# francescobrigante/Audio-Style-Transfer

Measured on AMD Instinct MI355X. Metric: audio-seconds/sec/node (train step, 4s@22.05kHz pairs), higher is better.
Workload: dtype bf16; 1 GPU; configs[1]: batch=8 4 s clips per GPU (S=2, x=(B,S,2,287,597)), full train2 step: STFT + CQT front-end from resident waveforms, encoders+decoder+discriminator, all losses, D and G phases, grad clip, Adam; global_batch=8, parallelism=dp1, hip_graph=True, dp_semantics=per-rank BN and batch-coupled losses

## Files before the change

### audio-style-transfer_amd/ast_amd/ops.py

```python
from __future__ import annotations

import functools
import math

import torch

from . import _lib, config
from ._lib import Gather, check, dcode, lib, ptr, stream


@functools.lru_cache(maxsize=None)
def const_tensor(values, dtype, device):
    return torch.tensor(values, dtype=dtype, device=device)


def pad8(c: int) -> int:
    return (c + 7) // 8 * 8


def _tap(dh, dw, wt):
    return (dh + 64) | ((dw + 64) << 8) | (wt << 16)


def _mk(N, Hs, Ws, Cs, Hm, Wm, sh, sw, oh, ow, Hd, Wd, Cd, dsh, dsw, doh, dow, taps, wtaps):
# ... 19 lines not shown
        th = [((ph + pad - kh) // stride, kh) for kh in range(k) if (ph + pad - kh) % stride == 0]
        Hm = (Hd - ph + stride - 1) // stride
        for pw in range(stride):
            tw = [((pw + pad - kw) // stride, kw) for kw in range(k) if (pw + pad - kw) % stride == 0]
            Wm = (Wd - pw + stride - 1) // stride
            if Hm <= 0 or Wm <= 0:
                continue
            taps = tuple((dh, dw, kh * k + kw) for dh, kh in th for dw, kw in tw)
            out.append(_mk(N, Hs, Ws, Cs, Hm, Wm, 1, 1, 0, 0, Hd, Wd, Cd, stride, stride, ph, pw, taps, k * k))
    return tuple(out)


PROFILE = None


def _gemm_cost(g, esize, wgrad=False):
    M = g.N * g.Hm * g.Wm
    K = g.ntaps * g.Cs
    flops = 2.0 * M * g.Cd * K
    if wgrad:
        nbytes = (M * g.Cd + g.N * g.Hs * g.Ws * g.Cs) * esize + g.Cd * K * 4
    else:
        src_pix = min(g.N * g.Hs * g.Ws, M * max(g.ntaps, 1))
        nbytes = (src_pix * g.Cs + M * g.Cd + g.Cd * K) * esize
    return flops, nbytes


def _igemm_config(g, dt):
    import ctypes
    out = (ctypes.c_int32 * 5)()
    check(lib().ast_igemm_plan(g, dt, ctypes.byref(out)), "ast_igemm_plan")
    if out[2] < 0:
        return f"patch{-out[0]}r{'(rows,' + str(-out[3]) + 'frag)' if out[3] < 0 else ''},{out[1]}ch,slab{-out[2]}B"
    return f"{out[0]}x{out[1]},k{out[2] * 16}B" + (f",split{out[3]}" if out[3] > 1 else "") + (f",kg{out[4]}" if out[4] > 1 else "")


_ws_cache = {}


def _ws_need(g, dt):
    key = (id(g), dt)
    v = _ws_cache.get(key)
    if v is None:
        v = int(lib().ast_igemm_ws_floats(g, dt))
        if v < 0:
            check(-1, "ast_igemm_ws_floats")
        _ws_cache[key] = v
    return v


STAT_SLOTS = 64


def stat_slots(C):
    s = STAT_SLOTS
    while s > 8 and s * C > 4096:
        s //= 2
    return s


def _slot_flags(slots):
    return 0 if slots == 64 else ((slots.bit_length() - 1) << 8)


class _StatArena:
    CAP = 1 << 24
# ... 13 lines not shown
        a[0].zero_()
        a[1] = 0
    t = a[0][a[1]:a[1] + int(n)]
    a[1] += n64
    a[2] = max(a[2], a[1])
    return t


def stat_arena_reset(device):
    a = _StatArena.by_device.get(torch.device(device))
    if a is None or a[2] == 0:
        return
    if config.fused_finalize or _SyncBN.active:
        a[0][:a[2]].zero_()
    a[1] = 0


def stats_fusable(g, dt):
    return _ws_need(g, dt) == 0


class BNLink:
    __slots__ = ("x", "scale", "shift", "relu", "table", "filled", "slots")

    def __init__(self):
        self.x = self.scale = self.shift = self.table = None
        self.relu, self.filled, self.slots = True, False, STAT_SLOTS


def in_stats_fusable(g, dt):
    import ctypes
    out = (ctypes.c_int32 * 5)()
    check(lib().ast_igemm_plan(g, dt, ctypes.byref(out)), "ast_igemm_plan")
    return out[2] != 0 and _ws_need(g, dt) == 0


def _igemm(src, wgt, bias, dst, g, flags=0, stats=None, bn=None, per_image=False):
    if PROFILE is not None:
        e0, e1 = torch.cuda.Event(enable_timing=True), torch.cuda.Event(enable_timing=True)
        e0.record()
    need = _ws_need(g, dcode(src.dtype))
    if bn is not None:
        assert need == 0 and flags == 0
        check(lib().ast_igemm_bn(ptr(src), ptr(wgt), ptr(bias), ptr(dst), g, dcode(src.dtype), 16 | (0 if bn.relu else 32) | _slot_flags(bn.slots), ptr(bn.table),
                                 bn.table.numel(), ptr(bn.x), ptr(bn.scale), ptr(bn.shift), stream()), "ast_igemm_bn")
    else:
        if stats is not None:
            assert need == 0 and flags == 0
            ws, need, flags = stats, stats.numel(), (8 | 64 if per_image else 8 | _slot_flags(stats.numel() // (2 * g.Cd)))
        else:
            ws = _clean_scratch(need, src.device) if need > 0 else None
            flags |= 4 if need > 0 else 0
        check(lib().ast_igemm(ptr(src), ptr(wgt), ptr(bias), ptr(dst), g, dcode(src.dtype), flags, ptr(ws), need,
                              stream()), "ast_igemm")
    if PROFILE is not None:
        e1.record()
        fl, by = _gemm_cost(g, src.element_size())
        dt = "bf16" if src.dtype == torch.bfloat16 else "f32"
        PROFILE.append((f"igemm_kernel<{dt},{_igemm_config(g, dcode(src.dtype))}>", fl, by, e0, e1))


class _WgradStream:
    stream = None
    dirty = False


def _wgrad(dy, src, dwp, g, replicas=1, pw=None):
# ... 1108 lines not shown
```

### audio-style-transfer_amd/csrc/igemm.hip

```cpp
#include "gemm_common.h"

namespace {


__device__ __forceinline__ int swz(int row, int c) { return ((c + (((row >> 3) & 1) << 1)) & 3) << 4; }

template <typename T>
struct EpiCtx {
  T* dst; const float* bias; float* ws; const T* bn_x; const float* bn_scale; const float* bn_shift;
  int HWm; float rcp_hw, rcp_w; bool accumulate, relu, stats, bstats, bn_relu;
};

template <typename T, int TN, int MODE>
__device__ __forceinline__ void epi_store_m(const EpiCtx<T>& ec, const ast_gather_t& g, const f32x4 (&col)[TN], const size_t pix, const int co0,
                                            float (&st1)[TN][4], float (&st2)[TN][4]) {
  T* drow = ec.dst + pix * g.Cd;
#pragma unroll
  for (int i = 0; i < TN; ++i) {
    const int co = co0 + i * 16;
    if (co >= g.Cd) continue;
    float v[4];
#pragma unroll
    for (int r = 0; r < 4; ++r) v[r] = col[i][r];
    if (ec.bias) {
// ... 310 lines not shown
  const bool split = gridDim.z > 1;
  const bool stats = (flags & 8) && !split;
  const bool bstats = (flags & 16) && !split;
  const bool bn_relu = !(flags & 32);
  EpiCtx<T> ec{dst, bias, ws, bn_x, bn_scale, bn_shift, HWm, rcp_hw, rcp_w, accumulate, relu, stats, bstats, bn_relu};
  float st1[TN][4], st2[TN][4];
#pragma unroll
  for (int i = 0; i < TN; ++i)
#pragma unroll
    for (int r = 0; r < 4; ++r) { st1[i][r] = 0.f; st2[i][r] = 0.f; }
#pragma unroll
  for (int j = 0; j < TM; ++j) {
    const int m = bm0 + wm * WTM + j * 16 + fr;
    if (m >= M_end) continue;
    if (split) {
#pragma unroll
      for (int i = 0; i < TN; ++i) {
        const int co = bn0 + wn * WTN + i * 16 + fq * 4;
        if (co >= g.Cd) continue;
#pragma unroll
        for (int r = 0; r < 4; ++r) unsafeAtomicAdd(ws + (size_t)m * g.Cd + co + r, acc[i][j][r]);
      }
      continue;
    }
    f32x4 col[TN];
#pragma unroll
    for (int i = 0; i < TN; ++i) col[i] = acc[i][j];
    epi_pixel<T, TN>(ec, g, col, m, bn0 + wn * WTN + fq * 4, st1, st2);
  }
  float* const red = (KG == 1 && WN == 1) ? reinterpret_cast<float*>(lds_all) : nullptr;
  if (stats || bstats) epi_flush<T, TN>(ec, g, st1, st2, per_image ? ~img : (tix & stat_slot_mask(flags)), bn0 + wn * WTN, fr, fq, red);
}

template <typename T, int TN, int NKS>
__global__ __launch_bounds__(256) void igemm_direct_kernel(const T* __restrict__ src, const T* __restrict__ wgt,
                                                           const float* __restrict__ bias, T* __restrict__ dst,
                                                           const ast_gather_t g, const int M, const int flags,
                                                           float* __restrict__ ws, const int cpc_shift,
                                                           const unsigned src_bytes, const unsigned wgt_bytes,
                                                           const float rcp_hw, const float rcp_w,
                                                           const T* __restrict__ bn_x, const float* __restrict__ bn_scale,
                                                           const float* __restrict__ bn_shift, const int jt) {
  constexpr int E = 16 / sizeof(T), ES = sizeof(T);
  constexpr unsigned OOB = 0x80000000u;
  using frag = typename Mma<T>::frag;
  __shared__ int taptab[AST_MAX_TAPS];
  const int lane = threadIdx.x & 63, wave = threadIdx.x >> 6;
  const int fr = lane & 15, fq = lane >> 4;
  const int BMW = jt * 16, BM = 4 * BMW;
  const int MT = (M + BM - 1) / BM, NT = (g.Cd + TN * 16 - 1) / (TN * 16);
  const int chunk = gridDim.x >> 3;
  const int tix = (blockIdx.x & 7) * chunk + (blockIdx.x >> 3);
  if (tix >= MT * NT) return;
  const int ntile = tix / MT;
  const int bm0 = (tix - ntile * MT) * BM + wave * BMW, bn0 = ntile * TN * 16;
#pragma unroll
  for (int t = 0; t < AST_MAX_TAPS; ++t)
    if ((int)threadIdx.x == t) taptab[t] = g.tap[t];
  __syncthreads();
  const int cpc = g.Cs / E, nchunks = g.ntaps * cpc;
  const int nks = (nchunks + 3) >> 2;
  const int HWm = g.Hm * g.Wm;
  const __amdgpu_buffer_rsrc_t srcR = __builtin_amdgcn_make_buffer_rsrc((void*)src, 0, src_bytes, 0x00020000);
  const __amdgpu_buffer_rsrc_t wgtR = __builtin_amdgcn_make_buffer_rsrc((void*)wgt, 0, wgt_bytes, 0x00020000);

  int sdelta[NKS], tdh[NKS], tdw[NKS];
  unsigned woff[NKS];
#pragma unroll
  for (int ks = 0; ks < NKS; ++ks) {
    const int kc = ks * 4 + fq;
    const bool kval = kc < nchunks;
    const int t = kval ? (cpc_shift >= 0 ? (kc >> cpc_shift) : kc / cpc) : 0;
    const int c0b = (kc - t * cpc) * 16;
    int dh, dw, wt;
    decode_tap(taptab[t], dh, dw, wt);
    sdelta[ks] = (dh * g.Ws + dw) * g.Cs * ES + c0b;
    tdh[ks] = kval ? dh : (1 << 20);
    tdw[ks] = dw;
    woff[ks] = kval ? (unsigned)(wt * g.Cs * ES + c0b) : OOB;
  }
  frag wreg[TN][NKS];
#pragma unroll
  for (int i = 0; i < TN; ++i) {
    const int co = bn0 + i * 16 + fr;
    const unsigned rowoff = co < g.Cd ? (unsigned)(co * g.wtaps * g.Cs * ES) : OOB;
#pragma unroll
    for (int ks = 0; ks < NKS; ++ks)
      wreg[i][ks] = __builtin_bit_cast(frag, __builtin_amdgcn_raw_buffer_load_b128(wgtR, (rowoff != OOB && woff[ks] != OOB) ? rowoff + woff[ks] : OOB, 0, 0));
  }

  const bool accumulate = flags & 1, relu = flags & 2, stats = flags & 8, bstats = flags & 16, bn_relu = !(flags & 32);
  EpiCtx<T> ec{dst, bias, ws, bn_x, bn_scale, bn_shift, HWm, rcp_hw, rcp_w, accumulate, relu, stats, bstats, bn_relu};
  float st1[TN][4], st2[TN][4];
#pragma unroll
  for (int i = 0; i < TN; ++i)
#pragma unroll
    for (int r = 0; r < 4; ++r) { st1[i][r] = 0.f; st2[i][r] = 0.f; }

  auto load_pix = [&](int j, u32x4 (&xr)[NKS], int& dpix) __attribute__((always_inline)) {
    const int m = bm0 + j * 16 + fr;
    const bool valid = j < jt && m < M;
    const int mm = valid ? m : 0;
    const int n = fdiv(mm, HWm, rcp_hw), rem = mm - n * HWm;
    const int hm = fdiv(rem, g.Wm, rcp_w), wq = rem - hm * g.Wm;
    const int hs0 = valid ? hm * g.sh + g.oh : -(1 << 20);
    const int ws0 = wq * g.sw + g.ow;
    const int roff = (((n * g.Hs + (valid ? hs0 : 0)) * g.Ws + ws0) * g.Cs) * ES;
    dpix = (n * g.Hd + hm * g.dsh + g.doh) * g.Wd + (wq * g.dsw + g.dow);
#pragma unroll
    for (int ks = 0; ks < NKS; ++ks) {
      const bool ok = (unsigned)(hs0 + tdh[ks]) < (unsigned)g.Hs && (unsigned)(ws0 + tdw[ks]) < (unsigned)g.Ws;
      xr[ks] = __builtin_amdgcn_raw_buffer_load_b128(srcR, ok ? (unsigned)(roff + sdelta[ks]) : OOB, 0, 0);
    }
  };
  auto compute = [&](int j, const u32x4 (&xr)[NKS], const int dpix) __attribute__((always_inline)) {
    f32x4 acc[TN];
#pragma unroll
    for (int i = 0; i < TN; ++i) acc[i] = f32x4{0.f, 0.f, 0.f, 0.f};
#pragma unroll
    for (int ks = 0; ks < NKS; ++ks) {
      if (ks < nks) {
        const frag xf = __builtin_bit_cast(frag, xr[ks]);
#pragma unroll
        for (int i = 0; i < TN; ++i) acc[i] = Mma<T>::run(wreg[i][ks], xf, acc[i]);
      }
    }
    const int m = bm0 + j * 16 + fr;
    if (m < M) epi_store<T, TN>(ec, g, acc, (size_t)dpix, bn0 + fq * 4, st1, st2);
  };

  u32x4 xa[NKS], xb[NKS];
  int pa, pb;
  load_pix(0, xa, pa);
  for (int j = 0; j < jt; j += 2) {
    load_pix(j + 1, xb, pb);
    compute(j, xa, pa);
    load_pix(j + 2, xa, pa);
    if (j + 1 < jt) compute(j + 1, xb, pb);
  }
  __shared__ float red[(TN + 1) / 2 * 256];
  if (stats || bstats) epi_flush<T, TN>(ec, g, st1, st2, tix & stat_slot_mask(flags), bn0, fr, fq, red);
}

template <typename T>
__global__ __launch_bounds__(256) void splitk_finish_kernel(float* __restrict__ ws, const float* __restrict__ bias,
                                                            T* __restrict__ dst, const ast_gather_t g, const int M, const int flags) {
  const int c4 = g.Cd >> 2;
  const int HWm = g.Hm * g.Wm;
  const size_t total = (size_t)M * c4;
  for (size_t i = (size_t)blockIdx.x * 256 + threadIdx.x; i < total; i += (size_t)gridDim.x * 256) {
    const int m = (int)(i / c4), co = (int)(i % c4) * 4;
    const int n = m / HWm, rem = m - n * HWm;
    const int hm = rem / g.Wm, wq = rem - hm * g.Wm;
    const size_t pix = (size_t)(n * g.Hd + hm * g.dsh + g.doh) * g.Wd + (wq * g.dsw + g.dow);
    f32x4* wp = reinterpret_cast<f32x4*>(ws + (size_t)m * g.Cd + co);
    const f32x4 a = *wp;
    *wp = f32x4{0.f, 0.f, 0.f, 0.f};
    float v[4] = {a[0], a[1], a[2], a[3]};
    if (bias) for (int r = 0; r < 4; ++r) v[r] += bias[co + r];
    store4<T>(dst + pix * g.Cd + co, v, flags & 1, flags & 2);
  }
}

constexpr int PC_MAXPL = 8;

#ifdef AST_STAMPS
__device__ unsigned long long ast_stamps[16384 * 8];
#define PC_STAMP(k) do { if (threadIdx.x == 0 && tix < 16384) ast_stamps[tix * 8 + (k)] = (k) >= 6 ? wall_clock64() : __builtin_readcyclecounter(); } while (0)
#else
#define PC_STAMP(k) do { } while (0)
#endif
struct PconvPlan { int TH, TWF, PH, PW, dhmin, dwmin, tiles_h, tiles_w, nct, lds, rows, tm, wall; unsigned m_nct, m_per_img, m_tiles_w, m_pw20, m_twf, m_twf20; unsigned long long tapq[3]; };
__host__ __device__ __forceinline__ unsigned pc_magic(int d) { return d <= 1 ? 0u : (unsigned)((0x100000000ull + (unsigned)d - 1) / (unsigned)d); }
__device__ __forceinline__ int pc_div(int n, int d, unsigned m) { return d == 1 ? n : (int)__umulhi((unsigned)n, m); }
__device__ __forceinline__ int pc_div20(int n, unsigned m20) { return (int)(__umul24((unsigned)n, m20) >> 20); }

template <int SLB> __device__ __forceinline__ int pc_h(int p) { return SLB == 128 ? (p & 7) : ((p >> 1) & 3); }

typedef __attribute__((ext_vector_type(2))) unsigned int u32x2;
__device__ __forceinline__ f32x4 pc_as_f32x4(u32x4 u) {
  return __builtin_bit_cast(f32x4, u);
}
template <typename T>
__device__ __forceinline__ f32x4 pc_load4(__amdgpu_buffer_rsrc_t r, unsigned voff, int imm) {
  if constexpr (sizeof(T) == 4) {
    return pc_as_f32x4(__builtin_amdgcn_raw_buffer_load_b128(r, voff + (unsigned)imm, 0, 0));
  } else {
    const u32x2 u = __builtin_amdgcn_raw_buffer_load_b64(r, voff + (unsigned)imm, 0, 0);
    const u32x4 w{u.x << 16, u.x & 0xffff0000u, u.y << 16, u.y & 0xffff0000u};
    return __builtin_bit_cast(f32x4, w);
  }
}
template <typename T>
__device__ __forceinline__ void pc_store4(__amdgpu_buffer_rsrc_t r, unsigned voff, int imm, f32x4 v) {
  if constexpr (sizeof(T) == 4) {
    __builtin_amdgcn_raw_buffer_store_b128(__builtin_bit_cast(u32x4, v), r, voff + (unsigned)imm, 0, 0);
  } else {
    const bf16x4 q{(bf16_t)v[0], (bf16_t)v[1], (bf16_t)v[2], (bf16_t)v[3]};
    __builtin_amdgcn_raw_buffer_store_b64(__builtin_bit_cast(u32x2, q), r, voff + (unsigned)imm, 0, 0);
  }
}

template <typename T, int SLB, int TM, int TN, bool WALL>
__global__ __launch_bounds__(256, (WALL ? 2 : (TM * TN <= 8 ? 4 : 2))) void pconv_kernel(const T* __restrict__ src, const T* __restrict__ wgt, const float* __restrict__ bias,
                                                    T* __restrict__ dst, const ast_gather_t g, const PconvPlan pp, const int flags,
                                                    float* __restrict__ ws, const unsigned src_bytes, const unsigned wgt_bytes,
                                                    const T* __restrict__ bn_x, const float* __restrict__ bn_scale,
                                                    const float* __restrict__ bn_shift) {
  constexpr int ES = sizeof(T);
  constexpr int CPP = SLB / 16;
  constexpr int BN = TN * 16;
  constexpr int NWL = (BN * CPP + 255) / 256;
  constexpr int KS = SLB / 64;
  constexpr unsigned OOB = 0x80000000u;
  using frag = typename Mma<T>::frag;
  extern __shared__ __attribute__((aligned(16))) unsigned char pl[];
  const int patch_bytes = pp.PH * pp.PW * SLB;
  unsigned char* wbuf = pl + patch_bytes;

  const int tid = threadIdx.x, lane = tid & 63, wave = tid >> 6;
  const int fr = lane & 15, fq = lane >> 4;
  const int chunk = gridDim.x >> 3;
  const int tix = (blockIdx.x & 7) * chunk + (blockIdx.x >> 3);
  const int per_img = pp.tiles_h * pp.tiles_w;
  if (tix >= g.N * per_img * pp.nct) return;
  PC_STAMP(0); PC_STAMP(7);
  const int st = pc_div(tix, pp.nct, pp.m_nct), ct = tix - st * pp.nct;
  const int n = pc_div(st, per_img, pp.m_per_img), r = st - n * per_img;
  const int th = pc_div(r, pp.tiles_w, pp.m_tiles_w), tw = r - th * pp.tiles_w;
  const int TWP = pp.rows ? g.Wm : pp.TWF * 16;
  const int hm0 = th * pp.TH, wm0 = tw * TWP;
  const int bn0 = ct * BN;
// ... 377 lines not shown
  const int E = dtype == AST_BF16 ? 8 : 4;
  const int nchunks = g.ntaps * (g.Cs / E);
  IgemmPlan p;
  if (g.Cd > 64) { p.bm = 64; p.bn = (M >= 30000) ? 128 : 64; }
  else if (g.Cd > 32) { p.bm = 64; p.bn = 64; }
  else if (g.Cd > 16) { p.bn = 32; p.bm = M >= 4096 ? 128 : 64; }
  else { p.bn = 16; p.bm = M >= 4096 ? 128 : 64; }
  p.kch = (p.bn >= 64 && nchunks >= 16) ? 8 : 4;
  const int KT = (nchunks + p.kch - 1) / p.kch;
  const long blocks = (long)((M + p.bm - 1) / p.bm) * ((g.Cd + p.bn - 1) / p.bn);
  p.nsplit = 1;
  p.kgroups = 1;
  static const long kg_blocks = getenv("AST_IGEMM_KG_BLOCKS") ? atol(getenv("AST_IGEMM_KG_BLOCKS")) : 400;
  static const int kg_kch = getenv("AST_IGEMM_KG_KCH") ? atoi(getenv("AST_IGEMM_KG_KCH")) : 8;
  if (p.bm == 64 && p.bn == 64 && blocks < kg_blocks && KT >= 16) { p.kgroups = 4; p.kch = kg_kch == 4 ? 4 : 8; }
  else if (blocks < 200 && KT >= 16 && (long)M * g.Cd <= (1L << 20)) p.nsplit = blocks < 120 ? 4 : 2;
  p.depth = 2;
  if (const char* f = getenv("AST_IGEMM_FORCE")) {
    int a, b, c, d, e = 0;
    const int nf = sscanf(f, "%d,%d,%d,%d,%d", &a, &b, &c, &d, &e);
    if (nf >= 4) { p.bm = a; p.bn = b; p.kch = c; p.nsplit = std::max(1, d); p.depth = 2; p.kgroups = 1; }
    if (nf >= 5) p.kgroups = (e == 4 && a == 64 && b == 64) ? 4 : 1;
  }
  {
    const int KT2 = (nchunks + p.kch - 1) / p.kch;
    p.nsplit = std::max(1, std::min(p.nsplit, std::max(1, KT2)));
    p.kt_per_split = (KT2 + p.nsplit - 1) / p.nsplit;
    p.nsplit = KT2 > 0 ? (KT2 + p.kt_per_split - 1) / p.kt_per_split : 1;
  }
  if (p.kt_per_split < 1) p.kt_per_split = 1;
  return p;
}

bool direct_ok(const ast_gather_t& g, const IgemmPlan& p, int dtype) {
  static const bool enabled = !(getenv("AST_IGEMM_DIRECT") && atoi(getenv("AST_IGEMM_DIRECT")) == 0);
  const int E = dtype == AST_BF16 ? 8 : 4;
  const int nchunks = g.ntaps * (g.Cs / E);
  static const int max_cd = getenv("AST_IGEMM_DIRECT_CD") ? atoi(getenv("AST_IGEMM_DIRECT_CD")) : 16;
  static const int max_chunks = getenv("AST_IGEMM_DIRECT_CHUNKS") ? atoi(getenv("AST_IGEMM_DIRECT_CHUNKS")) : 12;
  if ((long)g.N * g.Hd * g.Wd >= (1L << 31)) return false;
  return enabled && g.Cd <= std::min(max_cd, 32) && nchunks <= std::min(max_chunks, 12) && p.nsplit == 1 && p.kgroups == 1 &&
         !getenv("AST_IGEMM_FORCE");
}
int direct_jt(int M) {
  static const int env = getenv("AST_IGEMM_DIRECT_JT") ? atoi(getenv("AST_IGEMM_DIRECT_JT")) : 0;
  if (env > 0) return std::min(env, 64);
  return std::max(1, std::min(8, M / (64 * 2048)));
}

template <typename T, int TN, int NKS>
int launch_direct(const void* src, const void* wgt, const float* bias, void* dst, const ast_gather_t& g, int M, int flags, float* ws,
                  const IgemmPlan& p, hipStream_t s) {
  const int E = 16 / sizeof(T), cpc = g.Cs / E;
  int shift = -1;
  if ((cpc & (cpc - 1)) == 0) { shift = 0; while ((1 << shift) < cpc) ++shift; }
  const int jt = direct_jt(M);
  const int tiles = ((M + 64 * jt - 1) / (64 * jt)) * ((g.Cd + TN * 16 - 1) / (TN * 16));
  const unsigned src_bytes = (unsigned)((size_t)g.N * g.Hs * g.Ws * g.Cs * sizeof(T));
  const unsigned wgt_bytes = (unsigned)((size_t)g.Cd * g.wtaps * g.Cs * sizeof(T));
  hipLaunchKernelGGL((igemm_direct_kernel<T, TN, NKS>), dim3((tiles + 7) / 8 * 8), dim3(256), 0, s, (const T*)src, (const T*)wgt, bias, (T*)dst, g,
                     M, flags, ws, shift, src_bytes, wgt_bytes, 1.0f / (float)(g.Hm * g.Wm), 1.0f / (float)g.Wm, (const T*)p.bn_x, p.bn_scale,
                     p.bn_shift, jt);
  AST_CHECK_LAUNCH();
  return 0;
}

template <typename T>
int dispatch_direct(const void* src, const void* wgt, const float* bias, void* dst, const ast_gather_t& g, int M, int flags, float* ws,
                    const IgemmPlan& p, hipStream_t s) {
  const int nks = (g.ntaps * (g.Cs / (16 / (int)sizeof(T))) + 3) / 4;
#define AST_DK(TN_, K_) return launch_direct<T, TN_, K_>(src, wgt, bias, dst, g, M, flags, ws, p, s)
  if (g.Cd <= 16) { if (nks <= 1) AST_DK(1, 1); if (nks <= 2) AST_DK(1, 2); AST_DK(1, 3); }
  if (nks <= 1) AST_DK(2, 1); if (nks <= 2) AST_DK(2, 2); AST_DK(2, 3);
#undef AST_DK
}

template <typename T, int BM, int BN, int WM, int WN, int KCH, int D, int KG, bool UT>
int launch_igemm_ut(const void* src, const void* wgt, const float* bias, void* dst, const ast_gather_t& g, int M, int flags,
                 float* ws, const IgemmPlan& p, hipStream_t s) {
  constexpr int LDS = KG * 2 * (KCH / 4) * (BM + BN) * 64 + 64;
  static_assert(KG == 1 || (KG - 1) * (BM / 16) * (BN / 16) / 4 * 256 * 16 <= KG * 2 * (KCH / 4) * (BM + BN) * 64, "reduce buffer fits");
  static bool attr_set = false;
  if (!attr_set) {
    AST_HIP(hipFuncSetAttribute((const void*)igemm_kernel<T, BM, BN, WM, WN, KCH, D, KG, UT>, hipFuncAttributeMaxDynamicSharedMemorySize, LDS));
    attr_set = true;
  }
  const int E = 16 / sizeof(T);
  const int cpc = g.Cs / E;
  int shift = -1;
  if ((cpc & (cpc - 1)) == 0) { shift = 0; while ((1 << shift) < cpc) ++shift; }
  const int mtiles = (flags & 64) ? g.N * ((g.Hm * g.Wm + BM - 1) / BM) : (M + BM - 1) / BM;
  const int tiles = mtiles * ((g.Cd + BN - 1) / BN);
  dim3 grid((tiles + 7) / 8 * 8, 1, p.nsplit);
  if (p.nsplit > 1 && !(flags & 4)) AST_HIP(hipMemsetAsync(ws, 0, sizeof(float) * (size_t)M * g.Cd, s));
  const unsigned src_bytes = (unsigned)((size_t)g.N * g.Hs * g.Ws * g.Cs * sizeof(T));
  const unsigned wgt_bytes = (unsigned)((size_t)g.Cd * g.wtaps * g.Cs * sizeof(T));
  hipLaunchKernelGGL((igemm_kernel<T, BM, BN, WM, WN, KCH, D, KG, UT>), grid, dim3(256 * KG), LDS, s, (const T*)src, (const T*)wgt, bias, (T*)dst, g, M,
                     flags, ws, p.kt_per_split, shift, src_bytes, wgt_bytes, 1.0f / (float)(g.Hm * g.Wm), 1.0f / (float)g.Wm,
                     (const T*)p.bn_x, p.bn_scale, p.bn_shift);
  if (p.nsplit > 1) {
    const size_t total = (size_t)M * (g.Cd >> 2);
    hipLaunchKernelGGL((splitk_finish_kernel<T>), dim3((unsigned)std::min<size_t>((total + 255) / 256, 2048)), dim3(256), 0, s, ws, bias,
                       (T*)dst, g, M, flags);
  }
  AST_CHECK_LAUNCH();
  return 0;
}

template <typename T, int BM, int BN, int WM, int WN, int KCH, int D, int KG>
int launch_igemm(const void* src, const void* wgt, const float* bias, void* dst, const ast_gather_t& g, int M, int flags,
                 float* ws, const IgemmPlan& p, hipStream_t s) {
  const int cpc = g.Cs / (16 / (int)sizeof(T));
  if (cpc % KCH == 0) return launch_igemm_ut<T, BM, BN, WM, WN, KCH, D, KG, true>(src, wgt, bias, dst, g, M, flags, ws, p, s);
  return launch_igemm_ut<T, BM, BN, WM, WN, KCH, D, KG, false>(src, wgt, bias, dst, g, M, flags, ws, p, s);
}

}

extern "C" long ast_igemm_ws_floats(const ast_gather_t* gp, int dtype) {
  if (!gp || check_gather(gp, "ast_igemm_ws_floats")) return -1;
  const int M = gp->N * gp->Hm * gp->Wm;
  {
    PconvPlan pp; int slb = 0, tn = 0;
    if (plan_pconv(*gp, dtype, pp, slb, tn)) return 0;
  }
  const IgemmPlan p = plan_igemm(*gp, M, dtype);
  return p.nsplit > 1 ? (long)M * gp->Cd : 0;
}

extern "C" int ast_igemm_plan(const ast_gather_t* gp, int dtype, int* out5) {
  if (!gp || !out5 || check_gather(gp, "ast_igemm_plan")) return -1;
  const IgemmPlan p = plan_igemm(*gp, gp->N * gp->Hm * gp->Wm, dtype);
  out5[0] = p.bm; out5[1] = p.bn; out5[2] = p.kch; out5[3] = p.nsplit; out5[4] = p.kgroups;
  {
    PconvPlan pp; int slb = 0, tn = 0;
    if (plan_pconv(*gp, dtype, pp, slb, tn)) {
      out5[0] = -pp.TH; out5[1] = tn * 16; out5[2] = -slb; out5[3] = pp.rows ? -(pp.tm * 4) : 1; out5[4] = 1;
      return 0;
    }
  }
  if (direct_ok(*gp, p, dtype)) {
    out5[0] = 64 * direct_jt(gp->N * gp->Hm * gp->Wm); out5[1] = gp->Cd <= 16 ? 16 : 32; out5[2] = 0;
  }
  return 0;
}

extern "C" int ast_igemm_bn(const void* src, const void* wgt, const float* bias, void* dst, const ast_gather_t* gp,
                            int dtype, int flags, float* ws, long ws_floats, const void* bn_x, const float* bn_scale,
                            const float* bn_shift, void* stream) {
  if (int rc = check_gather(gp, "ast_igemm")) return rc;
  if (!src || !wgt || !dst) AST_FAIL("ast_igemm: null pointer");
  const ast_gather_t g = *gp;
  const int M = g.N * g.Hm * g.Wm;
  hipStream_t s = (hipStream_t)stream;
  IgemmPlan p = plan_igemm(g, M, dtype);
  p.bn_x = bn_x; p.bn_scale = bn_scale; p.bn_shift = bn_shift;
  {
    PconvPlan pp; int slb = 0, tn = 0;
    if (plan_pconv(g, dtype, pp, slb, tn)) {
      if ((flags & 16) && ((flags & 11) || !ws || ws_floats < (stat_slot_mask(flags) + 1L) * g.Cd * 3 || !bn_x || !bn_scale || !bn_shift))
        AST_FAIL("ast_igemm: fused BatchNorm-backward sums need plain stores, a zeroed [64][Cd][3] table and the layer's x / scale / shift");
      if ((flags & 8) && ((flags & 3) || !ws || ws_floats < ((flags & 64) ? (long)g.N : stat_slot_mask(flags) + 1L) * g.Cd * 2)) AST_FAIL("ast_igemm: fused channel statistics need plain stores and a zeroed [64][Cd][2] (per image: [N][Cd][2]) table");
#define AST_PC(S_, M_, N_) do { if (pp.wall) return launch_pconv<T, S_, M_, N_, true>(src, wgt, bias, dst, g, pp, flags, ws, bn_x, bn_scale, bn_shift, s); \
                                return launch_pconv<T, S_, M_, N_, false>(src, wgt, bias, dst, g, pp, flags, ws, bn_x, bn_scale, bn_shift, s); } while (0)
      AST_DISPATCH_T(dtype, {
        if (slb == 128 && pp.tm == 1) { if (tn == 4) AST_PC(128, 1, 4); AST_PC(128, 1, 2); }
        if (slb == 128 && pp.tm == 2) { if (tn == 4) AST_PC(128, 2, 4); AST_PC(128, 2, 2); }
        if (slb == 128) { if (tn == 4) AST_PC(128, 3, 4); AST_PC(128, 3, 2); }
        if (pp.tm == 2) { if (tn == 4) AST_PC(64, 2, 4); AST_PC(64, 2, 2); }
        if (pp.tm == 4) { if (tn == 4) AST_PC(64, 4, 4); AST_PC(64, 4, 2); }
        if (tn == 4) AST_PC(64, 3, 4); AST_PC(64, 3, 2);
      });
#undef AST_PC
    }
  }
  if (p.nsplit > 1) {
    if (flags & (8 | 16)) AST_FAIL("ast_igemm: fused statistics (flags 8 / 16) are not available for a split-K plan (ast_igemm_ws_floats > 0)");
    if (!ws || ws_floats < (long)M * g.Cd) AST_FAIL("ast_igemm: this plan splits K and needs a workspace of %ld floats (ast_igemm_ws_floats), got %ld", (long)M * g.Cd, ws ? ws_floats : 0L);
  }
  if ((flags & 16) && ((flags & 11) || !ws || ws_floats < (stat_slot_mask(flags) + 1L) * g.Cd * 3 || !bn_x || !bn_scale || !bn_shift))
    AST_FAIL("ast_igemm: fused BatchNorm-backward sums need plain stores, a zeroed [64][Cd][3] table and the layer's x / scale / shift");
  if ((flags & 8) && !(flags & 64) && ((flags & 3) || !ws || ws_floats < (stat_slot_mask(flags) + 1L) * g.Cd * 2))
    AST_FAIL("ast_igemm: fused channel statistics need plain stores and a zeroed [64][Cd][2] table");
  if (flags & 64) {
    if (!(flags & 8) || (flags & 3) || p.nsplit > 1 || direct_ok(g, p, dtype)) AST_FAIL("ast_igemm: per-image statistics (flag 64) need flag 8, plain stores and the gathered kernel (ast_igemm_plan: kch > 0, no split)");
    if (!ws || ws_floats < (long)g.N * g.Cd * 2) AST_FAIL("ast_igemm: per-image statistics need a zeroed [N][Cd][2] table");
  }
  if (direct_ok(g, p, dtype)) { AST_DISPATCH_T(dtype, { return dispatch_direct<T>(src, wgt, bias, dst, g, M, flags, ws, p, s); }); }
#define AST_IG(BM_, BN_, WM_, WN_, K_) return launch_igemm<T, BM_, BN_, WM_, WN_, K_, 2, 1>(src, wgt, bias, dst, g, M, flags, ws, p, s)
#define AST_IG4(BM_, BN_, WM_, WN_, K_) return launch_igemm<T, BM_, BN_, WM_, WN_, K_, 2, 4>(src, wgt, bias, dst, g, M, flags, ws, p, s)
  AST_DISPATCH_T(dtype, {
    if (p.bm == 128 && p.bn == 128) { if (p.kch == 8) AST_IG(128, 128, 2, 2, 8); else AST_IG(128, 128, 2, 2, 4); }
    if (p.bm == 128 && p.bn == 64) { if (p.kch == 8) AST_IG(128, 64, 2, 2, 8); else AST_IG(128, 64, 2, 2, 4); }
    if (p.bm == 64 && p.bn == 64 && p.kgroups == 4) { if (p.kch == 8) AST_IG4(64, 64, 2, 2, 8); else AST_IG4(64, 64, 2, 2, 4); }
    if (p.bm == 64 && p.bn == 64) { if (p.kch == 8) AST_IG(64, 64, 2, 2, 8); else AST_IG(64, 64, 2, 2, 4); }
    if (p.bm == 64 && p.bn == 128) { if (p.kch == 8) AST_IG(64, 128, 1, 4, 8); else AST_IG(64, 128, 1, 4, 4); }
    if (p.bm == 128 && p.bn == 32) AST_IG(128, 32, 4, 1, 4);
    if (p.bm == 128 && p.bn == 16) AST_IG(128, 16, 4, 1, 4);
    if (p.bm == 256 && p.bn == 32) AST_IG(256, 32, 4, 1, 4);
    if (p.bm == 64 && p.bn == 32) AST_IG(64, 32, 4, 1, 4);
    if (p.bm == 256 && p.bn == 16) AST_IG(256, 16, 4, 1, 4);
    AST_IG(64, 16, 4, 1, 4);
  });
#undef AST_IG
#undef AST_IG4
  return 0;
}

extern "C" int ast_igemm(const void* src, const void* wgt, const float* bias, void* dst, const ast_gather_t* gp,
                         int dtype, int flags, float* ws, long ws_floats, void* stream) {
  return ast_igemm_bn(src, wgt, bias, dst, gp, dtype, flags & ~48, ws, ws_floats, nullptr, nullptr, nullptr, stream);
}
```

Baseline: 5367 audio-seconds/sec.

## Replace direct igemm kernel with row-segment narrow conv kernel

Replaces the per-pixel direct conv kernel for narrow output channels (Cd 8/16/32) with a kernel where each wave walks 16-pixel tiles along an output row segment. Per-tap source offsets are hoisted per row, interior tiles skip bounds checks, and the epilogue uses buffer stores. For Cd=32 the weight fragments are staged in LDS instead of registers. The new path also handles 1x1 spatial cases via a canonicalised geometry and supports fused BN statistics. The risks are different occupancy and coverage, since Cd=32 now goes to the new kernel only when M is large, and new edge-handling paths.

New measurement: 5491 audio-seconds/sec, median of 6. 1.02x the previous value.

```diff
diff --git a/audio-style-transfer_amd/ast_amd/ops.py b/audio-style-transfer_amd/ast_amd/ops.py
--- a/audio-style-transfer_amd/ast_amd/ops.py
+++ b/audio-style-transfer_amd/ast_amd/ops.py
@@ -75,6 +75,8 @@
     check(lib().ast_igemm_plan(g, dt, ctypes.byref(out)), "ast_igemm_plan")
     if out[2] < 0:
         return f"patch{-out[0]}r{'(rows,' + str(-out[3]) + 'frag)' if out[3] < 0 else ''},{out[1]}ch,slab{-out[2]}B"
+    if out[2] == 0 and out[3] < 0:
+        return f"narrow{out[0]}x{out[1]}"
     return f"{out[0]}x{out[1]},k{out[2] * 16}B" + (f",split{out[3]}" if out[3] > 1 else "") + (f",kg{out[4]}" if out[4] > 1 else "")
 
 
@@ -154,7 +156,7 @@
     import ctypes
     out = (ctypes.c_int32 * 5)()
     check(lib().ast_igemm_plan(g, dt, ctypes.byref(out)), "ast_igemm_plan")
-    return out[2] != 0 and _ws_need(g, dt) == 0
+    return (out[2] != 0 or out[3] < 0) and _ws_need(g, dt) == 0
 
 
 def _igemm(src, wgt, bias, dst, g, flags=0, stats=None, bn=None, per_image=False):
diff --git a/audio-style-transfer_amd/csrc/igemm.hip b/audio-style-transfer_amd/csrc/igemm.hip
--- a/audio-style-transfer_amd/csrc/igemm.hip
+++ b/audio-style-transfer_amd/csrc/igemm.hip
@@ -366,116 +366,6 @@
   if (stats || bstats) epi_flush<T, TN>(ec, g, st1, st2, per_image ? ~img : (tix & stat_slot_mask(flags)), bn0 + wn * WTN, fr, fq, red);
 }
 
-template <typename T, int TN, int NKS>
-__global__ __launch_bounds__(256) void igemm_direct_kernel(const T* __restrict__ src, const T* __restrict__ wgt,
-                                                           const float* __restrict__ bias, T* __restrict__ dst,
-                                                           const ast_gather_t g, const int M, const int flags,
-                                                           float* __restrict__ ws, const int cpc_shift,
-                                                           const unsigned src_bytes, const unsigned wgt_bytes,
-                                                           const float rcp_hw, const float rcp_w,
-                                                           const T* __restrict__ bn_x, const float* __restrict__ bn_scale,
-                                                           const float* __restrict__ bn_shift, const int jt) {
-  constexpr int E = 16 / sizeof(T), ES = sizeof(T);
-  constexpr unsigned OOB = 0x80000000u;
-  using frag = typename Mma<T>::frag;
-  __shared__ int taptab[AST_MAX_TAPS];
-  const int lane = threadIdx.x & 63, wave = threadIdx.x >> 6;
-  const int fr = lane & 15, fq = lane >> 4;
-  const int BMW = jt * 16, BM = 4 * BMW;
-  const int MT = (M + BM - 1) / BM, NT = (g.Cd + TN * 16 - 1) / (TN * 16);
-  const int chunk = gridDim.x >> 3;
-  const int tix = (blockIdx.x & 7) * chunk + (blockIdx.x >> 3);
-  if (tix >= MT * NT) return;
-  const int ntile = tix / MT;
-  const int bm0 = (tix - ntile * MT) * BM + wave * BMW, bn0 = ntile * TN * 16;
-#pragma unroll
-  for (int t = 0; t < AST_MAX_TAPS; ++t)
-    if ((int)threadIdx.x == t) taptab[t] = g.tap[t];
-  __syncthreads();
-  const int cpc = g.Cs / E, nchunks = g.ntaps * cpc;
-  const int nks = (nchunks + 3) >> 2;
-  const int HWm = g.Hm * g.Wm;
-  const __amdgpu_buffer_rsrc_t srcR = __builtin_amdgcn_make_buffer_rsrc((void*)src, 0, src_bytes, 0x00020000);
-  const __amdgpu_buffer_rsrc_t wgtR = __builtin_amdgcn_make_buffer_rsrc((void*)wgt, 0, wgt_bytes, 0x00020000);
-
-  int sdelta[NKS], tdh[NKS], tdw[NKS];
-  unsigned woff[NKS];
-#pragma unroll
-  for (int ks = 0; ks < NKS; ++ks) {
-    const int kc = ks * 4 + fq;
-    const bool kval = kc < nchunks;
-    const int t = kval ? (cpc_shift >= 0 ? (kc >> cpc_shift) : kc / cpc) : 0;
-    const int c0b = (kc - t * cpc) * 16;
-    int dh, dw, wt;
-    decode_tap(taptab[t], dh, dw, wt);
-    sdelta[ks] = (dh * g.Ws + dw) * g.Cs * ES + c0b;
-    tdh[ks] = kval ? dh : (1 << 20);
-    tdw[ks] = dw;
-    woff[ks] = kval ? (unsigned)(wt * g.Cs * ES + c0b) : OOB;
-  }
-  frag wreg[TN][NKS];
-#pragma unroll
-  for (int i = 0; i < TN; ++i) {
-    const int co = bn0 + i * 16 + fr;
-    const unsigned rowoff = co < g.Cd ? (unsigned)(co * g.wtaps * g.Cs * ES) : OOB;
-#pragma unroll
-    for (int ks = 0; ks < NKS; ++ks)
-      wreg[i][ks] = __builtin_bit_cast(frag, __builtin_amdgcn_raw_buffer_load_b128(wgtR, (rowoff != OOB && woff[ks] != OOB) ? rowoff + woff[ks] : OOB, 0, 0));
-  }
-
-  const bool accumulate = flags & 1, relu = flags & 2, stats = flags & 8, bstats = flags & 16, bn_relu = !(flags & 32);
-  EpiCtx<T> ec{dst, bias, ws, bn_x, bn_scale, bn_shift, HWm, rcp_hw, rcp_w, accumulate, relu, stats, bstats, bn_relu};
-  float st1[TN][4], st2[TN][4];
-#pragma unroll
-  for (int i = 0; i < TN; ++i)
-#pragma unroll
-    for (int r = 0; r < 4; ++r) { st1[i][r] = 0.f; st2[i][r] = 0.f; }
-
-  auto load_pix = [&](int j, u32x4 (&xr)[NKS], int& dpix) __attribute__((always_inline)) {
-    const int m = bm0 + j * 16 + fr;
-    const bool valid = j < jt && m < M;
-    const int mm = valid ? m : 0;
-    const int n = fdiv(mm, HWm, rcp_hw), rem = mm - n * HWm;
-    const int hm = fdiv(rem, g.Wm, rcp_w), wq = rem - hm * g.Wm;
-    const int hs0 = valid ? hm * g.sh + g.oh : -(1 << 20);
-    const int ws0 = wq * g.sw + g.ow;
-    const int roff = (((n * g.Hs + (valid ? hs0 : 0)) * g.Ws + ws0) * g.Cs) * ES;
-    dpix = (n * g.Hd + hm * g.dsh + g.doh) * g.Wd + (wq * g.dsw + g.dow);
-#pragma unroll
-    for (int ks = 0; ks < NKS; ++ks) {
-      const bool ok = (unsigned)(hs0 + tdh[ks]) < (unsigned)g.Hs && (unsigned)(ws0 + tdw[ks]) < (unsigned)g.Ws;
-      xr[ks] = __builtin_amdgcn_raw_buffer_load_b128(srcR, ok ? (unsigned)(roff + sdelta[ks]) : OOB, 0, 0);
-    }
-  };
-  auto compute = [&](int j, const u32x4 (&xr)[NKS], const int dpix) __attribute__((always_inline)) {
-    f32x4 acc[TN];
-#pragma unroll
-    for (int i = 0; i < TN; ++i) acc[i] = f32x4{0.f, 0.f, 0.f, 0.f};
-#pragma unroll
-    for (int ks = 0; ks < NKS; ++ks) {
-      if (ks < nks) {
-        const frag xf = __builtin_bit_cast(frag, xr[ks]);
-#pragma unroll
-        for (int i = 0; i < TN; ++i) acc[i] = Mma<T>::run(wreg[i][ks], xf, acc[i]);
-      }
-    }
-    const int m = bm0 + j * 16 + fr;
-    if (m < M) epi_store<T, TN>(ec, g, acc, (size_t)dpix, bn0 + fq * 4, st1, st2);
-  };
-
-  u32x4 xa[NKS], xb[NKS];
-  int pa, pb;
-  load_pix(0, xa, pa);
-  for (int j = 0; j < jt; j += 2) {
-    load_pix(j + 1, xb, pb);
-    compute(j, xa, pa);
-    load_pix(j + 2, xa, pa);
-    if (j + 1 < jt) compute(j + 1, xb, pb);
-  }
-  __shared__ float red[(TN + 1) / 2 * 256];
-  if (stats || bstats) epi_flush<T, TN>(ec, g, st1, st2, tix & stat_slot_mask(flags), bn0, fr, fq, red);
-}
-
 template <typename T>
 __global__ __launch_bounds__(256) void splitk_finish_kernel(float* __restrict__ ws, const float* __restrict__ bias,
                                                             T* __restrict__ dst, const ast_gather_t g, const int M, const int flags) {
@@ -532,6 +422,190 @@
   } else {
     const bf16x4 q{(bf16_t)v[0], (bf16_t)v[1], (bf16_t)v[2], (bf16_t)v[3]};
     __builtin_amdgcn_raw_buffer_store_b64(__builtin_bit_cast(u32x2, q), r, voff + (unsigned)imm, 0, 0);
+  }
+}
+
+template <typename T, int TN, int NKS, int MODE>
+__device__ __forceinline__ void narrow_epi(const f32x4 (&acc)[TN], const __amdgpu_buffer_rsrc_t dstR, const __amdgpu_buffer_rsrc_t bnxR,
+                                           const unsigned doff, const bool pv, const f32x4 (&bias4)[TN], const f32x4 (&sc4)[TN],
+                                           const f32x4 (&sf4)[TN], const bool accumulate, const bool relu, const bool bn_relu,
+                                           float (&st1)[TN][4], float (&st2)[TN][4]) {
+  constexpr int ES = sizeof(T);
+#pragma unroll
+  for (int i = 0; i < TN; ++i) {
+    const unsigned off = doff + i * 16 * ES;
+    f32x4 v;
+#pragma unroll
+    for (int r = 0; r < 4; ++r) v[r] = acc[i][r] + bias4[i][r];
+    if constexpr (MODE == 1) {
+#pragma unroll
+      for (int r = 0; r < 4; ++r) {
+        const float q = pv ? (float)(T)v[r] : 0.f;
+        st1[i][r] += q; st2[i][r] += q * q;
+      }
+    }
+    if constexpr (MODE == 2) {
+      const f32x4 xv = pc_load4<T>(bnxR, off, 0);
+#pragma unroll
+      for (int r = 0; r < 4; ++r) {
+        const float q = (float)(T)v[r];
+        const float dz = (pv && (!bn_relu || __builtin_fmaf(xv[r], sc4[i][r], sf4[i][r]) > 0.f)) ? q : 0.f;
+        st1[i][r] += dz; st2[i][r] += dz * xv[r];
+      }
+    }
+    if (accumulate) {
+      const f32x4 o = pc_load4<T>(dstR, off, 0);
+#pragma unroll
+      for (int r = 0; r < 4; ++r) v[r] += o[r];
+    }
+    if (relu) {
+#pragma unroll
+      for (int r = 0; r < 4; ++r) v[r] = fmaxf(v[r], 0.f);
+    }
+    pc_store4<T>(dstR, off, 0, v);
+  }
+}
+
+struct NarrowGeo {
+  int nseg, segt, units, upw;
+  unsigned m_nseg, m_hm;
+  int dwmin, dwmax;
+  unsigned src_bytes, wgt_bytes, dst_bytes;
+};
+
+template <typename T, int TN, int NKS, int MODE>
+__global__ __launch_bounds__(256) void narrow_conv_kernel(const T* __restrict__ src, const T* __restrict__ wgt,
+                                                          const float* __restrict__ bias, T* __restrict__ dst,
+                                                          const ast_gather_t g, const NarrowGeo ng, const int flags,
+                                                          float* __restrict__ ws, const T* __restrict__ bn_x,
+                                                          const float* __restrict__ bn_scale, const float* __restrict__ bn_shift) {
+  constexpr int E = 16 / sizeof(T), ES = sizeof(T);
+  constexpr unsigned OOB = 0x80000000u;
+  using frag = typename Mma<T>::frag;
+  __shared__ int taptab[AST_MAX_TAPS];
+  const int lane = threadIdx.x & 63, wave = __builtin_amdgcn_readfirstlane(threadIdx.x >> 6);
+  const int fr = lane & 15, fq = lane >> 4;
+#pragma unroll
+  for (int t = 0; t < AST_MAX_TAPS; ++t)
+    if ((int)threadIdx.x == t) taptab[t] = g.tap[t];
+  __syncthreads();
+  const int cpc = g.Cs / E, nchunks = g.ntaps * cpc;
+  const __amdgpu_buffer_rsrc_t srcR = __builtin_amdgcn_make_buffer_rsrc((void*)src, 0, ng.src_bytes, 0x00020000);
+  const __amdgpu_buffer_rsrc_t wgtR = __builtin_amdgcn_make_buffer_rsrc((void*)wgt, 0, ng.wgt_bytes, 0x00020000);
+  const __amdgpu_buffer_rsrc_t dstR = __builtin_amdgcn_make_buffer_rsrc((void*)dst, 0, ng.dst_bytes, 0x00020000);
+  const __amdgpu_buffer_rsrc_t bnxR = __builtin_amdgcn_make_buffer_rsrc((void*)(MODE == 2 ? bn_x : dst), 0, ng.dst_bytes, 0x00020000);
+
+  int lsrc[NKS], tdh[NKS], tdw[NKS];
+  constexpr bool WL = TN == 2;
+  frag wreg[WL ? 1 : TN][NKS];
+  __shared__ u32x4 wlds[WL ? TN * NKS * 64 : 1];
+#pragma unroll
+  for (int ks = 0; ks < NKS; ++ks) {
+    const int kc = ks * 4 + fq;
+    const bool kval = kc < nchunks;
+    const int t = kval ? kc / cpc : 0;
+    const int c0b = (kc - t * cpc) * 16;
+    int dh, dw, wt;
+    decode_tap(taptab[t], dh, dw, wt);
+    lsrc[ks] = ((dh * g.Ws + dw + fr * g.sw) * g.Cs) * ES + c0b;
+    tdh[ks] = kval ? dh : (1 << 20);
+    tdw[ks] = dw + fr * g.sw;
+    const unsigned woff = (unsigned)(wt * g.Cs * ES + c0b);
+#pragma unroll
+    for (int i = 0; i < TN; ++i) {
+      const int co = i * 16 + fr;
+      const unsigned o = (kval && co < g.Cd) ? (unsigned)(co * g.wtaps * g.Cs * ES) + woff : OOB;
+      if constexpr (WL) {
+        if ((i * NKS + ks) % 4 == wave) wlds[(i * NKS + ks) * 64 + lane] = __builtin_amdgcn_raw_buffer_load_b128(wgtR, o, 0, 0);
+      } else {
+        wreg[i][ks] = __builtin_bit_cast(frag, __builtin_amdgcn_raw_buffer_load_b128(wgtR, o, 0, 0));
+      }
+    }
+  }
+  if constexpr (WL) __syncthreads();
+  const bool accumulate = flags & 1, relu = flags & 2, bn_relu = !(flags & 32);
+  f32x4 bias4[TN], sc4[TN], sf4[TN];
+  float st1[TN][4], st2[TN][4];
+#pragma unroll
+  for (int i = 0; i < TN; ++i) {
+    const int co = i * 16 + fq * 4;
+    const bool cv = co < g.Cd;
+    bias4[i] = (bias && cv) ? *reinterpret_cast<const f32x4*>(bias + co) : f32x4{0.f, 0.f, 0.f, 0.f};
+    if constexpr (MODE == 2) {
+      sc4[i] = cv ? *reinterpret_cast<const f32x4*>(bn_scale + co) : f32x4{0.f, 0.f, 0.f, 0.f};
+      sf4[i] = cv ? *reinterpret_cast<const f32x4*>(bn_shift + co) : f32x4{0.f, 0.f, 0.f, 0.f};
+    }
+#pragma unroll
+    for (int r = 0; r < 4; ++r) { st1[i][r] = 0.f; st2[i][r] = 0.f; }
+  }
+  const unsigned dlane = fq * 4 < g.Cd ? (unsigned)((fr * g.dsw * g.Cd + fq * 4) * ES) : OOB;
+  const int dtile = 16 * g.dsw * g.Cd * ES, stile = 16 * g.sw * g.Cs * ES;
+
+  for (int k = 0; k < ng.upw; ++k) {
+    const int u = (blockIdx.x * ng.upw + k) * 4 + wave;
+    if (u >= ng.units) break;
+    const int r = pc_div(u, ng.nseg, ng.m_nseg), s = u - r * ng.nseg;
+    const int n = pc_div(r, g.Hm, ng.m_hm), hm = r - n * g.Hm;
+    const int w0 = s * ng.segt * 16;
+    const int ntl = min(ng.segt, (g.Wm - w0 + 15) >> 4);
+    const int hs0 = hm * g.sh + g.oh, ws0 = w0 * g.sw + g.ow;
+    const int rowbase = ((n * g.Hs + hs0) * g.Ws + ws0) * g.Cs * ES;
+    unsigned base[NKS];
+#pragma unroll
+    for (int ks = 0; ks < NKS; ++ks) base[ks] = (unsigned)(hs0 + tdh[ks]) < (unsigned)g.Hs ? (unsigned)(rowbase + lsrc[ks]) : OOB;
+    const int dbase = ((n * g.Hd + hm * g.dsh + g.doh) * g.Wd + w0 * g.dsw + g.dow) * g.Cd * ES;
+
+    auto load = [&](int j, u32x4 (&xr)[NKS]) __attribute__((always_inline)) {
+      const int c0 = ws0 + j * 16 * g.sw;
+      const bool inner = c0 + ng.dwmin >= 0 && c0 + 15 * g.sw + ng.dwmax < g.Ws && w0 + j * 16 + 16 <= g.Wm;
+      const unsigned so = (unsigned)(j * stile);
+      if (inner) {
+#pragma unroll
+        for (int ks = 0; ks < NKS; ++ks) xr[ks] = __builtin_amdgcn_raw_buffer_load_b128(srcR, base[ks] + so, 0, 0);
+      } else {
+        const bool pv = w0 + j * 16 + fr < g.Wm;
+#pragma unroll
+        for (int ks = 0; ks < NKS; ++ks) {
+          const bool ok = pv && (unsigned)(c0 + tdw[ks]) < (unsigned)g.Ws;
+          xr[ks] = __builtin_amdgcn_raw_buffer_load_b128(srcR, ok ? base[ks] + so : OOB, 0, 0);
+        }
+      }
+    };
+    auto compute = [&](int j, const u32x4 (&xr)[NKS]) __attribute__((always_inline)) {
+      f32x4 acc[TN];
+#pragma unroll
+      for (int i = 0; i < TN; ++i) acc[i] = f32x4{0.f, 0.f, 0.f, 0.f};
+      int wl = lane;
+      if constexpr (WL) asm volatile("" : "+v"(wl));
+#pragma unroll
+      for (int ks = 0; ks < NKS; ++ks) {
+        const frag xf = __builtin_bit_cast(frag, xr[ks]);
+#pragma unroll
+        for (int i = 0; i < TN; ++i) {
+          if constexpr (WL) acc[i] = Mma<T>::run(__builtin_bit_cast(frag, wlds[(i * NKS + ks) * 64 + wl]), xf, acc[i]);
+          else acc[i] = Mma<T>::run(wreg[i][ks], xf, acc[i]);
+        }
+      }
+      const unsigned dt = dlane + (unsigned)(dbase + j * dtile);
+      if (w0 + j * 16 + 16 <= g.Wm) {
+        narrow_epi<T, TN, NKS, MODE>(acc, dstR, bnxR, dt, true, bias4, sc4, sf4, accumulate, relu, bn_relu, st1, st2);
+      } else {
+        const bool pv = w0 + j * 16 + fr < g.Wm;
+        narrow_epi<T, TN, NKS, MODE>(acc, dstR, bnxR, pv ? dt : OOB, pv, bias4, sc4, sf4, accumulate, relu, bn_relu, st1, st2);
+      }
+    };
+    u32x4 xa[NKS], xb[NKS];
+    load(0, xa);
+    for (int j = 0; j < ntl; j += 2) {
+      if (j + 1 < ntl) load(j + 1, xb);
+      compute(j, xa);
+      if (j + 2 < ntl) load(j + 2, xa);
+      if (j + 1 < ntl) compute(j + 1, xb);
+    }
+  }
+  if constexpr (MODE != 0) {
+    __shared__ float red[(TN + 1) / 2 * 256];
+    epi_flush<TN>(ws, MODE == 2, g.Cd, st1, st2, blockIdx.x & stat_slot_mask(flags), 0, fr, fq, red);
   }
 }
 
@@ -975,47 +1049,77 @@
   return p;
 }
 
-bool direct_ok(const ast_gather_t& g, const IgemmPlan& p, int dtype) {
+ast_gather_t narrow_canon(const ast_gather_t& g) {
+  ast_gather_t c = g;
+  if (g.Hs == 1 && g.Ws == 1 && g.Hm == 1 && g.Wm == 1 && g.Hd == 1 && g.Wd == 1 && g.ntaps == 1 && (g.tap[0] & 0xffff) == (64 | (64 << 8)) &&
+      g.oh == 0 && g.ow == 0 && g.doh == 0 && g.dow == 0) {
+    c.N = 1; c.Ws = c.Wm = c.Wd = g.N; c.sw = c.dsw = 1;
+  }
+  return c;
+}
+int narrow_form(const ast_gather_t& g0, const IgemmPlan& p, int dtype) {
+  const ast_gather_t g = narrow_canon(g0);
   static const bool enabled = !(getenv("AST_IGEMM_DIRECT") && atoi(getenv("AST_IGEMM_DIRECT")) == 0);
-  const int E = dtype == AST_BF16 ? 8 : 4;
+  if (!enabled || getenv("AST_IGEMM_FORCE") || p.nsplit != 1 || p.kgroups != 1) return 0;
+  const int E = dtype == AST_BF16 ? 8 : 4, ES = 16 / E;
   const int nchunks = g.ntaps * (g.Cs / E);
-  static const int max_cd = getenv("AST_IGEMM_DIRECT_CD") ? atoi(getenv("AST_IGEMM_DIRECT_CD")) : 16;
-  static const int max_chunks = getenv("AST_IGEMM_DIRECT_CHUNKS") ? atoi(getenv("AST_IGEMM_DIRECT_CHUNKS")) : 12;
-  if ((long)g.N * g.Hd * g.Wd >= (1L << 31)) return false;
-  return enabled && g.Cd <= std::min(max_cd, 32) && nchunks <= std::min(max_chunks, 12) && p.nsplit == 1 && p.kgroups == 1 &&
-         !getenv("AST_IGEMM_FORCE");
-}
-int direct_jt(int M) {
-  static const int env = getenv("AST_IGEMM_DIRECT_JT") ? atoi(getenv("AST_IGEMM_DIRECT_JT")) : 0;
-  if (env > 0) return std::min(env, 64);
-  return std::max(1, std::min(8, M / (64 * 2048)));
+  const long M = (long)g.N * g.Hm * g.Wm;
+  if ((long)g.N * g.Hd * g.Wd * g.Cd * ES >= (1L << 31)) return 0;
+  if ((g.Cd != 8 && g.Cd != 16 && g.Cd != 32) || g.Wm < 16) return 0;
+  const long tiles_row = (g.Wm + 15) / 16, units = (long)g.N * g.Hm * tiles_row;
+  if (units * std::max<long>(std::max<long>(tiles_row, g.Hm), 1) >= (1L << 32)) return 0;
+  if (nchunks > 12) return 0;
+  if (g.Cd <= 16) return 1;
+  return M >= 131072 ? 2 : 0;
+}
+NarrowGeo narrow_geo(const ast_gather_t& g, int esize) {
+  static const int env_segt = getenv("AST_NARROW_SEGT") ? atoi(getenv("AST_NARROW_SEGT")) : 0;
+  NarrowGeo ng;
+  const int tiles_row = (g.Wm + 15) / 16;
+  ng.segt = std::max(1, std::min(env_segt > 0 ? env_segt : 4, tiles_row));
+  ng.nseg = (tiles_row + ng.segt - 1) / ng.segt;
+  ng.units = g.N * g.Hm * ng.nseg;
+  ng.upw = std::max(1, std::min(8, ng.units / (4 * 2048)));
+  ng.m_nseg = pc_magic(ng.nseg); ng.m_hm = pc_magic(g.Hm);
+  ng.dwmin = 1 << 20; ng.dwmax = -(1 << 20);
+  for (int t = 0; t < g.ntaps; ++t) {
+    int dh, dw, wt;
+    dh = (g.tap[t] & 255) - 64; dw = ((g.tap[t] >> 8) & 255) - 64; wt = g.tap[t] >> 16; (void)dh; (void)wt;
+    ng.dwmin = std::min(ng.dwmin, dw); ng.dwmax = std::max(ng.dwmax, dw);
+  }
+  ng.src_bytes = (unsigned)((size_t)g.N * g.Hs * g.Ws * g.Cs * esize);
+  ng.wgt_bytes = (unsigned)((size_t)g.Cd * g.wtaps * g.Cs * esize);
+  ng.dst_bytes = (unsigned)((size_t)g.N * g.Hd * g.Wd * g.Cd * esize);
+  return ng;
 }
 
 template <typename T, int TN, int NKS>
-int launch_direct(const void* src, const void* wgt, const float* bias, void* dst, const ast_gather_t& g, int M, int flags, float* ws,
+int launch_narrow(const void* src, const void* wgt, const float* bias, void* dst, const ast_gather_t& g0, int flags, float* ws,
                   const IgemmPlan& p, hipStream_t s) {
-  const int E = 16 / sizeof(T), cpc = g.Cs / E;
-  int shift = -1;
-  if ((cpc & (cpc - 1)) == 0) { shift = 0; while ((1 << shift) < cpc) ++shift; }
-  const int jt = direct_jt(M);
-  const int tiles = ((M + 64 * jt - 1) / (64 * jt)) * ((g.Cd + TN * 16 - 1) / (TN * 16));
-  const unsigned src_bytes = (unsigned)((size_t)g.N * g.Hs * g.Ws * g.Cs * sizeof(T));
-  const unsigned wgt_bytes = (unsigned)((size_t)g.Cd * g.wtaps * g.Cs * sizeof(T));
-  hipLaunchKernelGGL((igemm_direct_kernel<T, TN, NKS>), dim3((tiles + 7) / 8 * 8), dim3(256), 0, s, (const T*)src, (const T*)wgt, bias, (T*)dst, g,
-                     M, flags, ws, shift, src_bytes, wgt_bytes, 1.0f / (float)(g.Hm * g.Wm), 1.0f / (float)g.Wm, (const T*)p.bn_x, p.bn_scale,
-                     p.bn_shift, jt);
+  const ast_gather_t g = narrow_canon(g0);
+  const NarrowGeo ng = narrow_geo(g, sizeof(T));
+  const int blocks = (ng.units + 4 * ng.upw - 1) / (4 * ng.upw);
+#define AST_NK(MODE_) hipLaunchKernelGGL((narrow_conv_kernel<T, TN, NKS, MODE_>), dim3(blocks), dim3(256), 0, s, (const T*)src, (const T*)wgt, \
+                                         bias, (T*)dst, g, ng, flags, ws, (const T*)p.bn_x, p.bn_scale, p.bn_shift)
+  if (flags & 8) AST_NK(1);
+  else if (flags & 16) AST_NK(2);
+  else AST_NK(0);
+#undef AST_NK
   AST_CHECK_LAUNCH();
   return 0;
 }
 
 template <typename T>
-int dispatch_direct(const void* src, const void* wgt, const float* bias, void* dst, const ast_gather_t& g, int M, int flags, float* ws,
+int dispatch_narrow(const void* src, const void* wgt, const float* bias, void* dst, const ast_gather_t& g, int flags, float* ws,
                     const IgemmPlan& p, hipStream_t s) {
   const int nks = (g.ntaps * (g.Cs / (16 / (int)sizeof(T))) + 3) / 4;
-#define AST_DK(TN_, K_) return launch_direct<T, TN_, K_>(src, wgt, bias, dst, g, M, flags, ws, p, s)
-  if (g.Cd <= 16) { if (nks <= 1) AST_DK(1, 1); if (nks <= 2) AST_DK(1, 2); AST_DK(1, 3); }
-  if (nks <= 1) AST_DK(2, 1); if (nks <= 2) AST_DK(2, 2); AST_DK(2, 3);
-#undef AST_DK
+#define AST_NW(TN_) do { switch (nks) { \
+    case 1: return launch_narrow<T, TN_, 1>(src, wgt, bias, dst, g, flags, ws, p, s); \
+    case 2: return launch_narrow<T, TN_, 2>(src, wgt, bias, dst, g, flags, ws, p, s); \
+    default: return launch_narrow<T, TN_, 3>(src, wgt, bias, dst, g, flags, ws, p, s); } } while (0)
+  if (g.Cd <= 16) AST_NW(1);
+  AST_NW(2);
+#undef AST_NW
 }
 
 template <typename T, int BM, int BN, int WM, int WN, int KCH, int D, int KG, bool UT>
@@ -1082,8 +1186,9 @@
       return 0;
     }
   }
-  if (direct_ok(*gp, p, dtype)) {
-    out5[0] = 64 * direct_jt(gp->N * gp->Hm * gp->Wm); out5[1] = gp->Cd <= 16 ? 16 : 32; out5[2] = 0;
+  if (const int nf = narrow_form(*gp, p, dtype)) {
+    const NarrowGeo ng = narrow_geo(narrow_canon(*gp), dtype == AST_BF16 ? 2 : 4);
+    out5[0] = 16 * ng.segt; out5[1] = gp->Cd <= 16 ? 16 : 32; out5[2] = 0; out5[3] = nf == 2 ? -1 : 1;
   }
   return 0;
 }
@@ -1126,10 +1231,10 @@
   if ((flags & 8) && !(flags & 64) && ((flags & 3) || !ws || ws_floats < (stat_slot_mask(flags) + 1L) * g.Cd * 2))
     AST_FAIL("ast_igemm: fused channel statistics need plain stores and a zeroed [64][Cd][2] table");
   if (flags & 64) {
-    if (!(flags & 8) || (flags & 3) || p.nsplit > 1 || direct_ok(g, p, dtype)) AST_FAIL("ast_igemm: per-image statistics (flag 64) need flag 8, plain stores and the gathered kernel (ast_igemm_plan: kch > 0, no split)");
+    if (!(flags & 8) || (flags & 3) || p.nsplit > 1 || narrow_form(g, p, dtype) == 1) AST_FAIL("ast_igemm: per-image statistics (flag 64) need flag 8, plain stores and the gathered kernel (ast_igemm_plan: kch > 0, or the wide narrow form, no split)");
     if (!ws || ws_floats < (long)g.N * g.Cd * 2) AST_FAIL("ast_igemm: per-image statistics need a zeroed [N][Cd][2] table");
   }
-  if (direct_ok(g, p, dtype)) { AST_DISPATCH_T(dtype, { return dispatch_direct<T>(src, wgt, bias, dst, g, M, flags, ws, p, s); }); }
+  if (!(flags & 64) && narrow_form(g, p, dtype)) { AST_DISPATCH_T(dtype, { return dispatch_narrow<T>(src, wgt, bias, dst, g, flags, ws, p, s); }); }
 #define AST_IG(BM_, BN_, WM_, WN_, K_) return launch_igemm<T, BM_, BN_, WM_, WN_, K_, 2, 1>(src, wgt, bias, dst, g, M, flags, ws, p, s)
 #define AST_IG4(BM_, BN_, WM_, WN_, K_) return launch_igemm<T, BM_, BN_, WM_, WN_, K_, 2, 4>(src, wgt, bias, dst, g, M, flags, ws, p, s)
   AST_DISPATCH_T(dtype, {
```
